# foubari/ratio_guided_Multimodal_FM

Measured on AMD Instinct MI355X. Metric: paired images/sec (MNIST32+SVHN, 100 Euler steps), higher is better.
Workload: dtype f32; 1 GPU; MNIST32 (1x32x32) + SVHN (3x32x32) pair, mc_feng guidance 0.5, 100 Euler steps, N_mc=256, batch 512 per GPU (BASELINE configs[2]; configs[3] at 8 GPUs); global_batch=512, parallelism=rows sharded over 1 rank(s); all_gather(MC set) + gather(outputs), step=one full sampling call (MC pre-phase + ratio + guided Euler loop + gather)

## Files before the change

### ratio_guided_multimodal_fm_amd/csrc/conv_mfma_hx2w.hip

```cpp
#include <stdlib.h>

#include <type_traits>

#include "conv_hx2_common.h"

namespace rgfm {

__global__ void hx2w_filter_transform_kernel(const float* w, float* u, int Cout, int Cin) {
  const size_t total = (size_t)Cout * Cin;
  for (size_t i = blockIdx.x * (size_t)blockDim.x + threadIdx.x; i < total; i += (size_t)gridDim.x * blockDim.x) {
    const float* g = w + i * 9;
    float t[4][3];
    for (int j = 0; j < 3; ++j) {
      t[0][j] = g[j];
      t[1][j] = 0.5f * (g[j] + g[3 + j] + g[6 + j]);
      t[2][j] = 0.5f * (g[j] - g[3 + j] + g[6 + j]);
      t[3][j] = g[6 + j];
    }
    for (int r = 0; r < 4; ++r) {
      u[i * 16 + r * 4 + 0] = t[r][0];
      u[i * 16 + r * 4 + 1] = 0.5f * (t[r][0] + t[r][1] + t[r][2]);
      u[i * 16 + r * 4 + 2] = 0.5f * (t[r][0] - t[r][1] + t[r][2]);
      u[i * 16 + r * 4 + 3] = t[r][2];
    }
  }
}

__device__ __forceinline__ void hx2w_split1(float v, unsigned short& h, unsigned short& l) {
  unsigned ph, pl;
  hsplit2(v, 0.f, ph, pl);
  h = (unsigned short)(ph & 0xffffu), l = (unsigned short)(pl & 0xffffu);
}

__global__ void hx2w_pack_kernel(const float* u, unsigned short* out, const float* hq, int Cout, int Cin) {
  const float sw = hq[2];
  const int nch = Cin / 16;
  const size_t total = (size_t)Cout * Cin * 16;
  for (size_t i = blockIdx.x * (size_t)blockDim.x + threadIdx.x; i < total; i += (size_t)gridDim.x * blockDim.x) {
    const int kk = (int)(i & 7), lane = (int)((i >> 3) & 63), nt = (int)((i >> 9) & 1), pos = (int)((i >> 10) & 15);
    const size_t r = i >> 14;
    const int ch = (int)(r % nch), cb = (int)(r / nch);
    const int co = cb * 64 + nt * 32 + (lane & 31), ci = ch * 16 + (lane >> 5) * 8 + kk;
    unsigned short h, l;
    hx2w_split1(sw * u[((size_t)co * Cin + ci) * 16 + pos], h, l);
    const size_t o = ((((((size_t)cb * nch + ch) * 16 + pos) * 2 + nt) * 2) * 64 + lane) * 8 + kk;
    out[o] = h, out[o + 512] = l;
  }
}

void hx2_scale_launch(const float* w, size_t n, float* hq, hipStream_t s);
void launch_pack_conv_hx2w(const float* w, void* out, float* hq, float* tmp, int Cout, int Cin, hipStream_t s) {
  hipLaunchKernelGGL(hx2w_filter_transform_kernel, dim3(256), dim3(256), 0, s, w, tmp, Cout, Cin);
  hx2_scale_launch(tmp, (size_t)Cout * Cin * 16, hq, s);
  hipLaunchKernelGGL(hx2w_pack_kernel, dim3(256), dim3(256), 0, s, tmp, (unsigned short*)out, hq, Cout, Cin);
}

constexpr int HX2W_RREC = 80;

template <int WL2>
__global__ __launch_bounds__(512, 2) void conv_mfma_hx2w_kernel(const ConvArgs a, const int num_tiles) {
  constexpr int W = 1 << WL2, TH = 256 / W, TX = W / 2, WR = W + 2, HR = TH + 2, HALO = HR * WR;
  constexpr int PW = WR / 2, PH = HR / 2, PSZ = PW * PH;
  constexpr int RBYTES = ((4 * PSZ * HX2W_RREC + 1023) / 1024) * 1024;
  constexpr int MAXIT = (HALO * 4 + 511) / 512;
  extern __shared__ __attribute__((aligned(16))) char smw[];
  char* const sV = smw + RBYTES;
  float* const sTab = reinterpret_cast<float*>(smw + 128 * 1024 + 64 * 32 * 8);

  const int tid = threadIdx.x, lane = tid & 63, wave = __builtin_amdgcn_readfirstlane((int)threadIdx.x >> 6);
  const int l31 = lane & 31, hp = lane >> 5;
  const TileGeom g = a.g;
  const int H = g.H;
  const int tile = (int)blockIdx.x;
  const int b0 = tile / g.tps, row0 = (tile - b0 * g.tps) * TH;
  const int cb = (int)blockIdx.y;
  const int cin = a.C0 + a.C1, nch = cin / KC;
  (void)num_tiles;

  const int q4 = tid & 3;
  int poff[MAXIT], rdst[MAXIT];
  unsigned okmask = 0u;
#pragma unroll
  for (int j = 0; j < MAXIT; ++j) {
    const int it = tid + 512 * j;
    poff[j] = 0, rdst[j] = 4 * PSZ * HX2W_RREC + q4 * 16;
    if (it < HALO * 4) {
      const int hpx = it >> 2;
      const int hy = hpx / WR, hx = hpx - hy * WR;
      const int y = row0 + hy - 1, x = hx - 1;
      const int rec = ((hy & 1) * 2 + (hx & 1)) * PSZ + (hy >> 1) * PW + (hx >> 1);
      rdst[j] = rec * HX2W_RREC + q4 * 16;
      if (y >= 0 && y < H && x >= 0 && x < W) {
        okmask |= 1u << j;
        poff[j] = (b0 * H + y) * W + x;
      }
    }
  }
  static_assert(RBYTES >= 4 * PSZ * HX2W_RREC + 64, "room for the trash record");
  f32x4 ra[MAXIT];
  float hmax = 0.f;
  auto issue_a = [&](int c) {
    const int ch0 = c * KC;
    const bool first = ch0 < a.C0;
    const float* src = first ? a.in0 + ch0 : a.in1 + (ch0 - a.C0);
    const unsigned cs = (unsigned)(first ? a.C0 : a.C1);
#pragma unroll
    for (int j = 0; j < MAXIT; ++j)
      ra[j] = *(const hx_gf32x4*)(src + (size_t)(__umul24((unsigned)poff[j], cs) + (unsigned)(q4 * 4)));
  };
  issue_a(0);

  if (a.gn_stats0) {
    const GnLane gn_lane(wave, lane, gn_waves_log2(cin >> 3), cin >> 3);
    if (gn_lane.row == 0) gn_table_row(a, gn_lane, b0, true, sTab, HX_SA);
  } else {
    for (int c = tid; c < cin; c += 512) {
      const float2 e = *reinterpret_cast<const float2*>(a.ab + ((size_t)b0 * cin + c) * 2);
      float2 o;
      o.x = HX_SA * e.x, o.y = HX_SA * e.y;
      *reinterpret_cast<float2*>(sTab + 2 * c) = o;
    }
  }

  auto commit_a = [&](int c) {
    const char* ep = reinterpret_cast<const char*>(sTab) + (c * KC + 4 * q4) * 8;
    const f32x4 e0 = *reinterpret_cast<const f32x4*>(ep), e1 = *reinterpret_cast<const f32x4*>(ep + 16);
    char* const rb = smw;
#pragma unroll
    for (int j = 0; j < MAXIT; ++j) {
      f32x4 v = ra[j];
      v.x = silu_scaled(fmaf(e0.x, v.x, e0.y));
      v.y = silu_scaled(fmaf(e0.z, v.y, e0.w));
      v.z = silu_scaled(fmaf(e1.x, v.z, e1.y));
      v.w = silu_scaled(fmaf(e1.z, v.w, e1.w));
      const float keep = ((okmask >> j) & 1u) ? 1.f : 0.f;
      v = v * keep;
      hmax = hx_absmax3(v.x, v.y, hmax);
      hmax = hx_absmax3(v.z, v.w, hmax);
      *reinterpret_cast<f32x4*>(rb + rdst[j]) = v;
    }
  };

  const int grp = wave >> 2;
  const int tt = tid & 63, tq = wave & 3;
  const int tty = tt / TX, ttx = tt - tty * TX;
  const int rbase = (tty * PW + ttx) * HX2W_RREC + tq * 16;
  const int vkey = (tt >> 2) & 3;
  const int vdst_h = grp * (8 * 64 * HRW) + tt * HRW + (((tq >> 1) ^ vkey) & 3) * 16 + (tq & 1) * 8;
  const int vdst_l = grp * (8 * 64 * HRW) + tt * HRW + (((2 + (tq >> 1)) ^ vkey) & 3) * 16 + (tq & 1) * 8;

  int aofs[2][2];
#pragma unroll
  for (int mt = 0; mt < 2; ++mt)
#pragma unroll
    for (int pl = 0; pl < 2; ++pl) aofs[mt][pl] = (32 * mt + l31) * HRW + (((2 * pl + hp) ^ ((l31 >> 2) & 3)) & 3) * 16;
  const char* const wbase = reinterpret_cast<const char*>(a.wpkw) + (size_t)cb * nch * (16 * 4096) + (size_t)(2 * wave) * 4096 + lane * 16;
  f16x8 bfr[2][2][2];
  auto issue_b = [&](int c) {
    const char* p = wbase + (size_t)c * (16 * 4096);
#pragma unroll
    for (int pi = 0; pi < 2; ++pi)
#pragma unroll
      for (int nt = 0; nt < 2; ++nt)
#pragma unroll
        for (int pl = 0; pl < 2; ++pl)
          bfr[pi][nt][pl] = __builtin_bit_cast(f16x8, *(const hx_gf32x4*)(p + pi * 4096 + nt * 2048 + pl * 1024));
  };

  f32x16 acc[2][2][2];
#pragma unroll
  for (int pi = 0; pi < 2; ++pi)
#pragma unroll
    for (int mt = 0; mt < 2; ++mt)
#pragma unroll
      for (int nt = 0; nt < 2; ++nt)
#pragma unroll
        for (int r = 0; r < 16; ++r) acc[pi][mt][nt][r] = 0.f;

  auto transform = [&](int c) {
    const char* const rb = smw + rbase;
    auto rd = [&](int i, int j) -> f32x4 {
      const int off = (((i & 1) * 2 + (j & 1)) * PSZ + (i >> 1) * PW + (j >> 1)) * HX2W_RREC;
      return *reinterpret_cast<const f32x4*>(rb + off);
    };
    struct P2 {
      hx_f32x2 lo, hi;
    };
    auto ld = [&](int i, int j) -> P2 {
      const f32x4 v = rd(i, j);
      return P2{hx_f32x2{v.x, v.y}, hx_f32x2{v.z, v.w}};
    };
    auto sub = [](const P2& x, const P2& y) { return P2{x.lo - y.lo, x.hi - y.hi}; };
    auto add = [](const P2& x, const P2& y) { return P2{x.lo + y.lo, x.hi + y.hi}; };
    P2 t0[4], t1[4];
    if (grp == 0) {
#pragma unroll
      for (int j = 0; j < 4; ++j) {
        const P2 d0 = ld(0, j), d1 = ld(1, j), d2 = ld(2, j);
        t0[j] = sub(d0, d2), t1[j] = add(d1, d2);
      }
    } else {
#pragma unroll
      for (int j = 0; j < 4; ++j) {
        const P2 d1 = ld(1, j), d2 = ld(2, j), d3 = ld(3, j);
        t0[j] = sub(d2, d1), t1[j] = sub(d1, d3);
      }
    }
#pragma unroll
    for (int r = 0; r < 2; ++r) {
      const P2* t = r ? t1 : t0;
      const P2 v[4] = {sub(t[0], t[2]), add(t[1], t[2]), sub(t[2], t[1]), sub(t[1], t[3])};
#pragma unroll
      for (int cc = 0; cc < 4; ++cc) {
        unsigned h0, l0, h1, l1;
        hsplit2(v[cc].lo.x, v[cc].lo.y, h0, l0);
        hsplit2(v[cc].hi.x, v[cc].hi.y, h1, l1);
        const hx_u32x2 ph = {h0, h1}, pl = {l0, l1};
        *reinterpret_cast<hx_u32x2*>(sV + vdst_h + (r * 4 + cc) * (64 * HRW)) = ph;
        *reinterpret_cast<hx_u32x2*>(sV + vdst_l + (r * 4 + cc) * (64 * HRW)) = pl;
      }
    }
  };
  auto multiply = [&]() {
#pragma unroll
    for (int pi = 0; pi < 2; ++pi) {
      const char* vp = sV + (2 * wave + pi) * (64 * HRW);
      f16x8 af[2][2];
#pragma unroll
      for (int mt = 0; mt < 2; ++mt)
#pragma unroll
        for (int pl = 0; pl < 2; ++pl) af[mt][pl] = *reinterpret_cast<const f16x8*>(vp + aofs[mt][pl]);
      hx_mma3<2>(acc[pi], af, bfr[pi]);
    }
  };

  __syncthreads();
#pragma unroll 1
  for (int c = 0; c < nch; ++c) {
    commit_a(c);
    issue_b(c);
    __syncthreads();
    issue_a(c + 1 < nch ? c + 1 : c);
    transform(c);
    __syncthreads();
    multiply();
  }
  if (!(4.f * hmax < HX_BIG)) atomicOr(a.range_flag, 1u);

  const float qinv = a.hqw[1];
  float* const sE = reinterpret_cast<float*>(smw);
  float* const sS = reinterpret_cast<float*>(smw + 128 * 1024);
  const bool sample_ok = b0 < a.B;
  const int et = tid >> 3, ecq = tid & 7;
  const int ety = et / TX, etx = et - ety * TX;
  const size_t pix = ((size_t)b0 * H + row0 + 2 * ety) * W + 2 * etx;
  auto pass = [&](auto nt_tag) {
    constexpr int nt = decltype(nt_tag)::value;
    __syncthreads();
#pragma unroll
    for (int pi = 0; pi < 2; ++pi)
#pragma unroll
      for (int mt = 0; mt < 2; ++mt) {
        float* e = sE + ((size_t)(2 * wave + pi) * 64 + 32 * mt) * 32 + l31;
#pragma unroll
        for (int r = 0; r < 16; ++r) e[((r & 3) + 8 * (r >> 2) + 4 * hp) * 32] = acc[pi][mt][nt][r];
      }
    __syncthreads();
    const int c = cb * 64 + nt * 32 + 4 * ecq;
    f32x4 add = *reinterpret_cast<const f32x4*>(a.bias + c);
    if (a.temb && sample_ok)
      add += *reinterpret_cast<const f32x4*>(a.temb + ((size_t)(a.temb_per_row ? b0 : 0) + (a.step_ptr ? (size_t)*a.step_ptr : 0)) * a.temb_stride + c);
    f32x4 mm[16];
#pragma unroll
    for (int p = 0; p < 16; ++p) mm[p] = *reinterpret_cast<const f32x4*>(sE + ((size_t)(p * 64 + et) * 32 + 4 * ecq));
    f32x4 s0[4], s1[4];
#pragma unroll
    for (int cc = 0; cc < 4; ++cc) {
      s0[cc] = mm[cc] + mm[4 + cc] + mm[8 + cc];
      s1[cc] = mm[4 + cc] - mm[8 + cc] - mm[12 + cc];
    }
    f32x4 y[4] = {s0[0] + s0[1] + s0[2], s0[1] - s0[2] - s0[3], s1[0] + s1[1] + s1[2], s1[1] - s1[2] - s1[3]};
#pragma unroll
    for (int i = 0; i < 4; ++i) {
      y[i] = y[i] * qinv + add;
      const size_t o = (pix + (i >> 1) * W + (i & 1)) * a.Cout + c;
      if (a.res_mode == 1 && sample_ok) y[i] += *reinterpret_cast<const f32x4*>(a.res0 + o);
      if (sample_ok) *reinterpret_cast<f32x4*>(a.out + o) = y[i];
    }
    if (a.small_check && a.range_flag && sample_ok) {
      float m = 0.f;
#pragma unroll
      for (int i = 0; i < 4; ++i) m = hx_absmax3(y[i].x, y[i].y, hx_absmax3(y[i].z, y[i].w, m));
      hx_small_flag(a.range_flag, m);
    }
    {
      const f32x4 mean = ((y[0] + y[1]) + (y[2] + y[3])) * 0.25f;
      f32x4 m2 = {0.f, 0.f, 0.f, 0.f};
#pragma unroll
      for (int i = 0; i < 4; ++i) m2 += (y[i] - mean) * (y[i] - mean);
      const f32x4 lo = {mean.x, m2.x, mean.y, m2.y}, hi = {mean.z, m2.z, mean.w, m2.w};
      float* sp = sS + ((size_t)et * 32 + 4 * ecq) * 2;
      *reinterpret_cast<f32x4*>(sp) = lo;
      *reinterpret_cast<f32x4*>(sp + 4) = hi;
    }
    __syncthreads();
    if (tid < 128 && a.stats_out && sample_ok) {
      const int part = tid >> 5, co = tid & 31;
      float2 sv[16];
#pragma unroll
      for (int k = 0; k < 16; ++k) sv[k] = *reinterpret_cast<const float2*>(sS + ((size_t)(16 * part + k) * 32 + co) * 2);
      double mean = 0.0, m2 = 0.0;
#pragma unroll
      for (int k = 0; k < 16; ++k) {
        const double d = (double)sv[k].x - mean;
        mean += d * (1.0 / (double)(k + 1));
        m2 += (double)sv[k].y + d * d * (4.0 * (double)k / (double)(k + 1));
      }
      const int gpart = (tile - b0 * g.tps) * 4 + part;
      float2 o;
      o.x = (float)mean, o.y = (float)m2;
      *reinterpret_cast<float2*>(a.stats_out + (((size_t)b0 * g.nparts + gpart) * a.Cout + cb * 64 + nt * 32 + co) * 2) = o;
    }
  };
  pass(std::integral_constant<int, 0>{});
  pass(std::integral_constant<int, 1>{});
}

static size_t hx2w_lds_bytes(const ConvArgs& a) {
  return (size_t)128 * 1024 + 64 * 32 * 8 + (size_t)(a.C0 + a.C1) * 8;
}

bool conv_hx2w_supported(const ConvArgs& a, int mode) {
  if (mode != CONV_S1 || !a.wpkw || !a.hqw || !a.range_flag) return false;
  const TileGeom& g = a.g;
  if (g.spt != 1 || (g.W != 16 && g.W != 32) || g.th * g.W != 256 || g.H % g.th != 0) return false;
  if (a.Hin != g.H || a.Win != g.W) return false;
  if (a.Cout % 64 != 0 || (a.C0 + a.C1) % KC != 0 || a.C0 % KC != 0) return false;
  if (a.res_mode == 2 || a.fin_ab || a.pout || a.pin0 || a.ep_scale || !a.out) return false;
  if (a.res_mode == 1 && a.R0 != a.Cout) return false;
  if (a.gn_stats0) {
    const int cin = a.C0 + a.C1;
    if (cin < 32 || cin % 8 != 0 || cin > 256 || a.gn_nparts0 > 16 || a.gn_g.nparts > 16) return false;
  } else if (!a.ab) {
    return false;
  }
  const size_t px = (size_t)a.B * a.g.HW;
  if (px >= (1u << 24) || px * (size_t)(a.C0 > a.Cout ? a.C0 : a.Cout) >= (1ull << 32)) return false;
  return hx2w_lds_bytes(a) <= 160 * 1024;
}

#define HX2W_FOR_ALL(X) X(4) X(5)

int conv_hx2w_init() {
  int rc = 0;
#define RAISEWN(WL) rc |= raise_lds_limit(&conv_mfma_hx2w_kernel<WL>, 160 * 1024);
  HX2W_FOR_ALL(RAISEWN)
#undef RAISEWN
  return rc;
}

bool launch_conv_hx2w(const ConvArgs& a, int mode, hipStream_t s) {
  if (mode != CONV_S1) return false;
  const int tiles = geom_num_tiles(a.g, a.B);
  const dim3 grid(tiles, a.Cout / 64);
  const size_t lds = hx2w_lds_bytes(a);
  const int wl = a.g.W == 16 ? 4 : 5;
#define LAUNCHWN(WL) \
  if (wl == (WL)) { hipLaunchKernelGGL((conv_mfma_hx2w_kernel<WL>), grid, dim3(512), lds, s, a, tiles); return true; }
  HX2W_FOR_ALL(LAUNCHWN)
#undef LAUNCHWN
  return false;
}
#undef HX2W_FOR_ALL

}
```

### ratio_guided_multimodal_fm_amd/csrc/rgfm_host.h

```cpp
#pragma once
#include "../../include/rgfm.h"

#include <hip/hip_runtime.h>

#include <algorithm>
#include <cmath>
#include <cstdarg>
#include <cstdio>
#include <cstdlib>
#include <cstring>
#include <string>
#include <vector>

#include "rgfm_kernels.h"

using namespace rgfm;

inline thread_local std::string g_err;

inline int fail(int code, const char* fmt, ...) {
  char buf[512];
  va_list ap;
  va_start(ap, fmt);
  vsnprintf(buf, sizeof(buf), fmt, ap);
// ... 89 lines not shown

struct Bump {
  char* base = nullptr;
  size_t off = 0;
  size_t cap = 0;
  bool dry = true;
  bool overflow = false;
  Bump() = default;
  Bump(void* ws, size_t ws_bytes) : base((char*)ws), cap(ws_bytes), dry(false) {}
  unsigned* u(size_t n) { return reinterpret_cast<unsigned*>(f(n)); }
  float* f(size_t nfloats) {
    const size_t bytes = (nfloats * sizeof(float) + 255) & ~(size_t)255;
    const size_t o = off;
    off += bytes;
    if (dry) return nullptr;
    if (off > cap) {
      overflow = true;
      return reinterpret_cast<float*>(base);
    }
    return reinterpret_cast<float*>(base + o);
  }
};

struct Tensor {
  float* data = nullptr;
  float* stats = nullptr;
  int C = 0, S = 0;
  void* p = nullptr;
  bool p_valid = false;
};

struct Cursor {
  size_t off = 0;
  size_t take(size_t n) {
    const size_t r = off;
    off += n;
    return r;
  }
};

struct HxImage {
  size_t off = 0;
  int hq = 0;
  bool present = false;
  bool ok = false;
  bool usable() const { return present && ok; }
};

struct ConvW {
  size_t w_raw = 0, b = 0;
  size_t w_pk = 0;
  size_t w_bx3 = 0;
  int cin = 0, cout = 0, taps = 9;
  HxImage hx;
  HxImage hx9;
  HxImage wino;
  HxImage t2;
};

struct WeightLayout {
  size_t n_params = 0, n_packed = 0, n_packed3 = 0, n_packedh = 0;
  int n_hq = 0;
};

struct Planner {
  Cursor raw, pk, p3, ph;
  int nhq = 0;
  HxImage image(size_t n_fp16, const HxImage* same_scale = nullptr) {
    HxImage i;
    i.off = ph.take(n_fp16), i.hq = same_scale ? same_scale->hq : nhq++, i.present = true;
    return i;
  }
  ConvW conv(int cin, int cout, int taps) {
    ConvW w;
    w.cin = cin, w.cout = cout, w.taps = taps;
    w.w_raw = raw.take((size_t)cout * cin * taps);
    w.b = raw.take(cout);
    w.w_pk = pk.take((size_t)cout * cin * taps);
    w.w_bx3 = p3.take((size_t)cout * cin * taps * 3);
    w.hx = image((size_t)cout * cin * taps * 2);
    return w;
  }
  WeightLayout layout() const { return {raw.off, pk.off, p3.off, ph.off, nhq}; }
};

struct ResW {
  int cin = 0, cout = 0;
  size_t n1w, n1b, n2w, n2b, tw, tb;
  ConvW c1, c2, sk;
  bool has_skip = false;
  int temb_off = 0;
};

inline int nt32_of(int cout) { return (cout % 64 == 0) ? 2 : 1; }

inline bool on_gfx950() {
  int dev = 0;
  if (hipGetDevice(&dev) != hipSuccess) return false;
  hipDeviceProp_t p;
  if (hipGetDeviceProperties(&p, dev) != hipSuccess) return false;
  return strncmp(p.gcnArchName, "gfx950", 6) == 0;
}

enum { CONV_ARITH_HX2 = 0, CONV_ARITH_BX3 = 1, CONV_ARITH_F32 = 2 };
struct Modes {
  int conv = CONV_ARITH_HX2;
  bool overlap = true, fuse_fin = true, gn_consumer = true;
  bool pipelined = true;
  bool quad = true;
  bool c8 = true;
  bool s2 = true;
  bool pfmt = true;
  bool wino = false;
  bool up_t2 = true;
  bool rev_hx2 = true;
  bool prephase = true;
  bool graph = false;
};
inline thread_local Modes g_modes;
inline void refresh_modes() {
  Modes m;
  const char* e = getenv("RGFM_CONV");
  if (e && strcmp(e, "bx3") == 0) m.conv = CONV_ARITH_BX3;
  else if (e && strcmp(e, "f32") == 0) m.conv = CONV_ARITH_F32;
  e = getenv("RGFM_OVERLAP");
  m.overlap = !(e && e[0] == '0');
  e = getenv("RGFM_FUSE_FIN");
  m.fuse_fin = !(e && e[0] == '0');
  e = getenv("RGFM_GN");
  m.gn_consumer = !(e && strcmp(e, "table") == 0);
  e = getenv("RGFM_HX2P");
  m.pipelined = !(e && e[0] == '0');
  e = getenv("RGFM_HX2Q");
  m.quad = !(e && e[0] == '0');
  e = getenv("RGFM_HX2S");
  m.s2 = !(e && e[0] == '0');
  e = getenv("RGFM_HX2C");
  m.c8 = !(e && e[0] == '0');
  e = getenv("RGFM_HX2D");
  m.pfmt = !(e && e[0] == '0');
  g_conv_tuning.hx2d_cut = e && e[0] == '1' ? 1 : (e && e[0] == '2' ? 2 : 3);
  e = getenv("RGFM_WINO");
  m.wino = e && e[0] == '1';
  e = getenv("RGFM_UP_T2");
  m.up_t2 = !(e && e[0] == '0');
  e = getenv("RGFM_REV_HX2");
  m.rev_hx2 = !(e && e[0] == '0');
  e = getenv("RGFM_GRAPH");
  m.graph = e && e[0] == '1';
  e = getenv("RGFM_PREPHASE_PRIO");
  m.prephase = !(e && e[0] == '0');
  g_modes = m;
  e = getenv("RGFM_WINO_W32");
  g_conv_tuning.wino_w32 = e ? atoi(e) : 0;
  g_conv_tuning.s2_f32 = getenv("RGFM_S2_F32") != nullptr;
  g_conv_tuning.f32_simple = getenv("RGFM_CONV_SIMPLE") != nullptr;
}

struct ModeScope {
  int saved;
  explicit ModeScope(int handle_mode) : saved(g_modes.conv) {
    if (handle_mode >= 0) g_modes.conv = handle_mode;
  }
  ~ModeScope() { g_modes.conv = saved; }
};

constexpr int MAX_DEVICES = 16;
struct DevState {
  bool init = false;
  int num_cus = 256;
  hipStream_t side = nullptr;
  void* zeros = nullptr;
  hipEvent_t fork = nullptr, join = nullptr;
  hipEvent_t pre_pace = nullptr;
  hipStream_t main = nullptr;
  hipEvent_t main_fork = nullptr, main_join = nullptr;
  hipEvent_t graph_done = nullptr;
  std::vector<std::pair<hipGraphExec_t, hipGraph_t>> graphs;
};
inline DevState g_dev[MAX_DEVICES];

inline DevState* cur_dev() {
  int dev = 0;
  if (hipGetDevice(&dev) != hipSuccess || dev < 0 || dev >= MAX_DEVICES) return nullptr;
  return g_dev[dev].init ? &g_dev[dev] : nullptr;
}

inline int ensure_init() {
  if (!on_gfx950()) return fail(RGFM_ENODEVICE, "librgfm_hip needs a gfx950 (MI355X) device; none is current");
  int dev = 0;
  HIP_TRY(hipGetDevice(&dev));
  if (dev < 0 || dev >= MAX_DEVICES) return fail(RGFM_EINVAL, "device ordinal %d out of range (max %d)", dev, MAX_DEVICES - 1);
  DevState& d = g_dev[dev];
  if (!d.init) {
    int rc = guid_apply_init();
    for (const ConvKernel& k : CONV_KERNELS) rc |= k.init();
    if (rc != 0) return fail(RGFM_EHIP, "hipFuncSetAttribute(MaxDynamicSharedMemorySize) failed");
    hipDeviceProp_t p;
    if (hipGetDeviceProperties(&p, dev) == hipSuccess) d.num_cus = p.multiProcessorCount;
    const char* e = getenv("RGFM_HX2P_HALF");
    g_conv_tuning.hx2p_half = e ? atoi(e) : d.num_cus;
    HIP_TRY(hipStreamCreateWithFlags(&d.side, hipStreamNonBlocking));
    HIP_TRY(hipMalloc(&d.zeros, 256));
    HIP_TRY(hipMemset(d.zeros, 0, 256));
    HIP_TRY(hipEventCreateWithFlags(&d.fork, hipEventDisableTiming));
    HIP_TRY(hipEventCreateWithFlags(&d.join, hipEventDisableTiming));
    HIP_TRY(hipEventCreateWithFlags(&d.graph_done, hipEventDisableTiming));
    HIP_TRY(hipStreamCreateWithFlags(&d.main, hipStreamNonBlocking));
    HIP_TRY(hipEventCreateWithFlags(&d.main_fork, hipEventDisableTiming));
    HIP_TRY(hipEventCreateWithFlags(&d.main_join, hipEventDisableTiming));
    HIP_TRY(hipEventCreateWithFlags(&d.pre_pace, hipEventDisableTiming));
    d.init = true;
  }
  return RGFM_OK;
}

inline bool hx2w_pays(const ConvArgs& c) {
  return c.wpkw != nullptr && c.C0 + c.C1 >= 128 && (!g_conv_tuning.wino_w32 || c.g.W == 32);
}

inline int conv_route(const ConvArgs& c, int mode) {
  if (c.pin0) return RGFM_ROUTE_HX2D;
  const bool hx2 = g_modes.conv == CONV_ARITH_HX2, pipe = hx2 && g_modes.pipelined;
  if (pipe && g_modes.wino && hx2w_pays(c) && conv_hx2w_supported(c, mode)) return RGFM_ROUTE_HX2W;
  if (pipe && g_modes.s2 && conv_hx2s_supported(c, mode)) return RGFM_ROUTE_HX2S;
  if (pipe && g_modes.c8 && conv_hx2c_supported(c, mode)) return RGFM_ROUTE_HX2C;
  if (pipe && g_modes.quad && conv_hx2q_supported(c, mode)) return RGFM_ROUTE_HX2Q;
  if (pipe && conv_hx2p_supported(c, mode)) return RGFM_ROUTE_HX2P;
  if (hx2 && conv_hx2_supported(c, mode)) return RGFM_ROUTE_HX2;
  if (g_modes.conv != CONV_ARITH_F32 && conv_bx3_supported(c, mode)) return RGFM_ROUTE_BX3;
  return RGFM_ROUTE_F32;
}

inline bool p_producer_ok(const ConvArgs& c, int mode) {
  if (!g_modes.pfmt) return false;
  const int route = conv_route(c, mode);
  if (route == RGFM_ROUTE_HX2C) return true;
  return route == RGFM_ROUTE_HX2P && mode == CONV_S1 && c.g.W == 16 && c.g.H == 16 && c.g.spt == 1 && c.g.tps == 1 &&
         (c.Cout == 64 || c.Cout == 128 || c.Cout == 256) && !c.ep_scale && !c.fin_ab;
}

inline bool launch_conv_on(int route, const ConvArgs& c, int mode, hipStream_t s) {
  const ConvKernel& k = CONV_KERNELS[route];
  if (k.launch(c, mode, s)) return true;
  fail(RGFM_EINVAL, "no %s instantiation for mode %d, Cout %d, %d x %d raster, res_mode %d", k.name, mode, c.Cout, c.g.H, c.g.W, c.res_mode);
  return false;
}

inline void launch_conv(const ConvArgs& c, int mode, hipStream_t s, int* routes = nullptr) {
  const int route = conv_route(c, mode);
  if (routes) {
    routes[route] += 1;
    if (mode == CONV_T2) routes[RGFM_ROUTE_T2] += 1;
  }
  launch_conv_on(route, c, mode, s);
}



inline int read_flag_word(unsigned* word, int* flagged, int reset, hipStream_t s) {
  if (!flagged) return fail(RGFM_EINVAL, "null output");
  *flagged = 0;
  if (!word) return RGFM_OK;
  unsigned v = 0;
  HIP_TRY(hipMemcpyAsync(&v, word, sizeof(v), hipMemcpyDeviceToHost, s));
  HIP_TRY(hipStreamSynchronize(s));
  *flagged = (int)v;
  if (reset && v) HIP_TRY(hipMemsetAsync(word, 0, sizeof(v), s));
  return RGFM_OK;
}
inline int alloc_flag_word(unsigned** word) {
  HIP_TRY(hipMalloc(word, 256));
  HIP_TRY(hipMemset(*word, 0, 256));
  return RGFM_OK;
}
inline int check_conv_mode(int mode) {
  if (mode < -1 || mode > CONV_ARITH_F32) return fail(RGFM_EINVAL, "conv mode must be RGFM_CONV_DEFAULT, _HX2, _BX3 or _F32");
  return RGFM_OK;
}


struct WeightStore : WeightLayout {
  float* params = nullptr;
  float* packed = nullptr;
  unsigned short* packed3 = nullptr;
  unsigned short* packedh = nullptr;
  float* hq = nullptr;
  unsigned* range_flag = nullptr;
  int conv_mode = -1;

  int alloc(const float* params_dev, bool with_range_flag, hipStream_t s) {
    if (hipMalloc(&params, n_params * sizeof(float)) != hipSuccess) return fail(RGFM_ENOMEM, "hipMalloc(params)");
    if (hipMalloc(&packed, (n_packed + 4) * sizeof(float)) != hipSuccess) return fail(RGFM_ENOMEM, "hipMalloc(packed)");
    if (hipMalloc(&packedh, (n_packedh + 8) * sizeof(unsigned short)) != hipSuccess) return fail(RGFM_ENOMEM, "hipMalloc(packedh)");
    if (hipMalloc(&hq, ((size_t)n_hq * 4 + 4) * sizeof(float)) != hipSuccess) return fail(RGFM_ENOMEM, "hipMalloc(hq)");
    if (with_range_flag && alloc_flag_word(&range_flag) != RGFM_OK) return fail(RGFM_ENOMEM, "hipMalloc(range flag)");
    if (n_packed3 && hipMalloc(&packed3, (n_packed3 + 8) * sizeof(unsigned short)) != hipSuccess)
      return fail(RGFM_ENOMEM, "hipMalloc(packed3)");
    if (hipMemcpyAsync(params, params_dev, n_params * sizeof(float), hipMemcpyDeviceToDevice, s) != hipSuccess)
      return fail(RGFM_EHIP, "hipMemcpyAsync(params)");
    return RGFM_OK;
  }
  void free() {
    for (void* p : {(void*)params, (void*)packed, (void*)packed3, (void*)packedh, (void*)hq, (void*)range_flag})
      if (p) (void)hipFree(p);
  }
};

inline int read_hx_flags(const WeightStore& st, const std::vector<HxImage*>& images, hipStream_t s) {
  std::vector<float> host((size_t)st.n_hq * 4);
  if (hipMemcpyAsync(host.data(), st.hq, host.size() * sizeof(float), hipMemcpyDeviceToHost, s) != hipSuccess ||
      hipStreamSynchronize(s) != hipSuccess)
    return fail(RGFM_EHIP, "reading the fp16 scale records failed");
  for (HxImage* i : images) i->ok = host[(size_t)i->hq * 4 + 3] != 0.f;
  return RGFM_OK;
}

inline bool norm_params_ok(const std::vector<float>& host, size_t gw, size_t gb, int C) {
  float mg = 0.f, mb = 0.f;
  for (int i = 0; i < C; ++i) mg = std::max(mg, std::fabs(host[gw + i])), mb = std::max(mb, std::fabs(host[gb + i]));
  if (!(mg <= 3.0e38f) || !(mb <= 3.0e38f)) return false;
  const float hi = 8.f * mg + mb, lo = std::max(mg, mb);
  return hi < 1024.f && lo >= 0.015625f;
}

struct NormGate {
  size_t gamma, beta;
  int C;
  HxImage* image;
};

inline int demote_by_norms(const WeightStore& st, const std::vector<NormGate>& gates, hipStream_t s) {
  std::vector<float> host(st.n_params);
  if (hipMemcpyAsync(host.data(), st.params, host.size() * sizeof(float), hipMemcpyDeviceToHost, s) != hipSuccess ||
      hipStreamSynchronize(s) != hipSuccess)
    return fail(RGFM_EHIP, "reading the parameters back failed");
  for (const NormGate& g : gates)
    if (!norm_params_ok(host, g.gamma, g.beta, g.C)) g.image->ok = false;
  return RGFM_OK;
}


struct rgfm_unet : WeightStore {
  rgfm_unet_desc d;
  float* freqs = nullptr;
  TimeLinear* lin_dev = nullptr;
  float* wtmp = nullptr;
  int mc = 0, temb = 0, nlin = 0, temb_total = 0;
  size_t te0w, te0b, te2w, te2b, icw, icb, onw, onb, ocw, ocb;
  size_t ocw_pk = 0;
  std::vector<ResW> enc, mid, dec;
  std::vector<ConvW> down, up;
  int final_ch = 0;
  bool trace = false;
  int wino_convs = 0;
  int p_handovers = 0;
  int routes[RGFM_ROUTE_SLOTS] = {};
  struct Act {
    float* data;
    int C, S;
    bool nchw;
  };
  std::vector<Act> acts;
};


inline size_t plan_unet(const rgfm_unet_desc& d, rgfm_unet* h) {
  Planner P;
  Cursor& c = P.raw;
  const int mc = d.model_channels, temb = 4 * mc;
  std::vector<ResW> enc, mid, dec;
// ... 530 lines not shown
```

### ratio_guided_multimodal_fm_amd/csrc/rgfm_kernels.h

```cpp
#pragma once
#include <hip/hip_runtime.h>
#include <stddef.h>
#include <stdint.h>

#include "../../include/rgfm.h"

namespace rgfm {

constexpr int KC = 16;
constexpr int LDP = 20;

struct TileGeom {
  int H, W, HW;
  int spt;
  int th;
  int tps;
  int nparts;
};

__host__ __device__ inline TileGeom make_geom(int H, int W) {
  TileGeom g;
  g.H = H;
  g.W = W;
  g.HW = H * W;
// ... 16 lines not shown
__host__ __device__ inline int geom_num_tiles(const TileGeom& g, int B) {
  return g.spt == 1 ? B * g.tps : (B + g.spt - 1) / g.spt;
}

__host__ __device__ inline int geom_part_count(const TileGeom& g, int part) {
  if (g.spt != 1) return g.HW;
  const int tile = part >> 2, w = part & 3;
  int rows = g.H - tile * g.th;
  if (rows > g.th) rows = g.th;
  int n = rows * g.W - 64 * w;
  return n < 0 ? 0 : (n > 64 ? 64 : n);
}

enum ConvMode { CONV_S1 = 0, CONV_S2 = 1, CONV_UP2 = 2, CONV_T2 = 3 };

struct ConvArgs {
  const float* in0;
  const float* in1;
  int C0, C1;
  int Hin, Win;
  const float* ab;
  const float* gn_stats0;
  const float* gn_stats1;
  const float* gn_gamma;
  const float* gn_beta;
  int gn_nparts0;
  TileGeom gn_g;
  const unsigned* in_amax;
  const void* pin0;
  const void* zeros;
  void* pout;
  const float* pn_gamma;
  const float* pn_beta;
  const float* wpk;
  const void* wpk3;
  const void* wskip3;
  const void* wpkh;
  const void* wskiph;
  const void* wpkh9;
  const float* hq;
  const float* hq_skip;
  unsigned* range_flag;
  int small_check;
  const float* bias;
  const float* temb;
  int temb_stride;
  int temb_per_row;
  const int* step_ptr;
  int res_mode;
  const float* res0;
  const float* res1;
  int R0, R1;
  const float* wskip;
  const float* skip_bias;
  const float* ep_scale;
  const float* ep_shift;
  int ep_nosilu;
  float* out;
  float* stats_out;
  float* fin_ab;
  unsigned* fin_counter;
  int fin_expected;
  const float* fin_stats1;
  int fin_C1;
  const float* fin_gamma;
  const float* fin_beta;
  const void* wpkw;
  const float* hqw;
  int B, Cout;
  TileGeom g;
  int halo_px;
};

inline int conv_halo_px(const ConvArgs& a) { return a.g.spt * (a.g.th + 2) * (a.g.W + 2); }
inline int conv_block_channels(int Cout) { return Cout % 128 == 0 ? 128 : (Cout % 64 == 0 ? 64 : 32); }
template <class Kernel>
inline int raise_lds_limit(Kernel* kernel, int bytes) {
  return (int)hipFuncSetAttribute(reinterpret_cast<const void*>(kernel), hipFuncAttributeMaxDynamicSharedMemorySize, bytes);
}

struct ConvInArgs {
  const float* x;
  const float* w;
  const float* bias;
  const float* ep_scale;
  const float* ep_shift;
  int ep_nosilu;
  float* out;
  float* stats_out;
  int B, C0;
  TileGeom g;
  unsigned* range_flag;
  int small_check;
};

struct ConvOutArgs {
  const float* in;
  const float* ab;
  const float* w;
  const float* bias;
  float* v_out;
  float* x_state;
  const float* x_base;
  float dt;
  int B, Cin;
  TileGeom g;
  int halo_px;
};

struct GnFinalizeArgs {
  const float* stats0;
  const float* stats1;
  int C0, C1, groups;
  const float* gamma;
  const float* beta;
  float* ab;
  int B;
  TileGeom g;
  int rep;
  float* mr;
};

struct TimeLinear {
  int w_off, b_off, cout, out_off;
};

struct TimeEmbedArgs {
  const float* params;
  const float* freqs;
  int mc, temb;
  int te0w, te0b, te2w, te2b;
  const TimeLinear* lin;
  int nlin;
  int total;
  const float* t_dev;
  int num_steps, step_begin;
  float* table;
  float* emb_out;
};


struct ConvTuning {
  int hx2p_half = 256;
  int hx2p_w4 = 0;
  int hx2q_min = 1024;
  int hx2q_target = 512;
  int hx2q_tpw = 0;
  int hx2q_cut = 0;
  int hx2q_all = 0;
  int hx2s_on = 1;
  int hx2c_on = 1;
  int hx2c_all = 0;
  int hx2d_cut = 3;
  int wino_w32 = 0;
  bool s2_f32 = false;
  bool f32_simple = false;
};
inline ConvTuning g_conv_tuning;

int conv_fin_expected(const ConvArgs& a, int mode);

int conv_mfma_init();
bool launch_conv_mfma(const ConvArgs& a, int mode, hipStream_t s);
size_t conv_mfma_lds_bytes(const ConvArgs& a);

bool conv_bx3_supported(const ConvArgs& a, int mode);
bool conv_bx3_gn_supported(const ConvArgs& a, int mode);
int conv_bx3_init();
bool launch_conv_bx3(const ConvArgs& a, int mode, hipStream_t s);
void launch_pack_conv_bx3(const float* w, void* out, int Cout, int Cin, int taps, hipStream_t s);
void launch_pack_deconv_bx3(const float* w, void* out, int Cin, int Cout, hipStream_t s);
void launch_pack_conv_bx3_s2(const float* w, void* out, int Cout, int Cin, hipStream_t s);

bool conv_hx2_supported(const ConvArgs& a, int mode);
bool conv_hx2_gn_supported(const ConvArgs& a, int mode);
int conv_hx2_init();
bool launch_conv_hx2(const ConvArgs& a, int mode, hipStream_t s);
void launch_pack_conv_hx2(const float* w, void* out, float* hq, int Cout, int Cin, int taps, int mode, hipStream_t s);
void launch_up2_as_deconv(const float* w, float* k, int Cout, int Cin, hipStream_t s);

bool conv_hx2p_supported(const ConvArgs& a, int mode);
int conv_hx2p_init();
bool launch_conv_hx2p(const ConvArgs& a, int mode, hipStream_t s);

bool conv_hx2q_supported(const ConvArgs& a, int mode);
int conv_hx2q_init();
bool launch_conv_hx2q(const ConvArgs& a, int mode, hipStream_t s);

bool conv_hx2s_supported(const ConvArgs& a, int mode);
int conv_hx2s_init();
bool launch_conv_hx2s(const ConvArgs& a, int mode, hipStream_t s);

bool conv_hx2c_supported(const ConvArgs& a, int mode);
int conv_hx2c_init();
bool launch_conv_hx2c(const ConvArgs& a, int mode, hipStream_t s);

bool conv_hx2d_supported(const ConvArgs& a, int mode);
int conv_hx2d_init();
bool launch_conv_hx2d(const ConvArgs& a, int mode, hipStream_t s);
void launch_hx_presplit(const float* in, const float* ab, void* pout, int B, int HW, int C, hipStream_t s);

bool conv_hx2w_supported(const ConvArgs& a, int mode);
int conv_hx2w_init();
bool launch_conv_hx2w(const ConvArgs& a, int mode, hipStream_t s);
void hx2_scale_launch(const float* w, size_t n, float* hq, hipStream_t s);
void launch_pack_conv_hx2w(const float* w, void* out, float* hq, float* tmp, int Cout, int Cin, hipStream_t s);

struct ConvKernel {
  const char* name;
  int (*init)();
  bool (*launch)(const ConvArgs& a, int mode, hipStream_t s);
};
inline constexpr ConvKernel CONV_KERNELS[RGFM_ROUTE_COUNT] = {
    {"hx2d", conv_hx2d_init, launch_conv_hx2d},
    {"hx2w", conv_hx2w_init, launch_conv_hx2w},
    {"hx2s", conv_hx2s_init, launch_conv_hx2s},
    {"hx2c", conv_hx2c_init, launch_conv_hx2c},
    {"hx2q", conv_hx2q_init, launch_conv_hx2q},
    {"hx2p", conv_hx2p_init, launch_conv_hx2p},
    {"hx2", conv_hx2_init, launch_conv_hx2},
    {"bx3", conv_bx3_init, launch_conv_bx3},
    {"f32", conv_mfma_init, launch_conv_mfma},
};
static_assert(RGFM_ROUTE_HX2D == 0 && RGFM_ROUTE_HX2W == 1 && RGFM_ROUTE_HX2S == 2 && RGFM_ROUTE_HX2C == 3 && RGFM_ROUTE_HX2Q == 4 &&
                  RGFM_ROUTE_HX2P == 5 && RGFM_ROUTE_HX2 == 6 && RGFM_ROUTE_BX3 == 7 && RGFM_ROUTE_F32 == 8,
              "CONV_KERNELS is written in RGFM_ROUTE_* order");

void launch_conv_in(const ConvInArgs& a, int cin, hipStream_t s);
void launch_conv_out(const ConvOutArgs& a, int cimg, hipStream_t s);
void launch_pack_conv_out(const float* w, float* out, int cimg, int Cin, hipStream_t s);
void launch_gn_finalize(const GnFinalizeArgs& a, hipStream_t s);
void launch_time_embed(const TimeEmbedArgs& a, int nt, hipStream_t s);
void launch_pack_conv(const float* w, float* out, int Cout, int Cin, int taps, int nt32, hipStream_t s);
void launch_pack_deconv(const float* w, float* out, int Cin, int Cout, int nt32, hipStream_t s);
void launch_permute_cols(const float* w, float* out, int rows, int C, int P, hipStream_t s);
void launch_permute_rows(const float* w, const float* b, float* wout, float* bout, int C, int P, int K, hipStream_t s);
void launch_fm_time_embed(const float* t_dev, int t_count, int num_steps, int step, const float* freqs, float* out,
                          int B, int dim, int stride, int col0, hipStream_t s);
void launch_nhwc_to_nchw(const float* in, float* out, int B, int C, int HW, hipStream_t s);
void launch_range_low_check(const float* in, int B, int HW, int C, unsigned* flag, hipStream_t s);

void launch_pool2(const float* in, const float* ab, float* out, int B, int H, int W, int C, hipStream_t s);
void launch_avgpool(const float* in, const float* ab, float* out, int B, int HW, int C, hipStream_t s);
void launch_linear_mfma(const float* x, const float* w, const float* b, float* y, int rows, int in,
                        int out, int x_stride, int y_stride, hipStream_t s);
void launch_linear_mfma_splitk(const float* x, const float* ab, int C, const float* w, const float* b, float* y,
                               float* part, int splits, int rows, int in, int out, int y_stride, hipStream_t s);
void launch_layernorm_silu(float* x, const float* w, const float* b, int rows, int n, hipStream_t s);
void launch_cross_ln_silu(const float* ux, const float* uy, const float* bias, const float* w, const float* b, float* out,
                          long long row0, int rows, int ny, int n, hipStream_t s);
void launch_cond_ln_silu(const float* ctx, const float* ut, const float* w, const float* b, float* u, float* a, int rows, int n,
                         hipStream_t s);
void launch_ratio_head(const float* x, const float* w, const float* b, float* out, int rows, int n,
                       int loss, int what, hipStream_t s);
void launch_bn_fold(const float* w, const float* b, const float* rm, const float* rv, float* scale,
                    float* shift, int C, hipStream_t s);

void launch_conv_weight_transpose(const float* w, float* wt, int Co, int Ci, hipStream_t s);
void launch_transpose2d(const float* w, float* wt, int rows, int cols, hipStream_t s);
void launch_fill(float* p, float v, size_t n, hipStream_t s);
void launch_fill_ab_identity(float* ab, size_t n_pairs, hipStream_t s);
void launch_grad_act(const float* g, const float* z, const float* scale, float* gz, int B, int S, int C, int mode, hipStream_t s,
                     unsigned* amax = nullptr);
void launch_grad_act_gn(const float* g, const float* z, const float* ab, float* gu, int B, int S, int C, int mode, hipStream_t s);
void launch_gn_bwd(float* gu, const float* z, const float* gamma, const float* mr, int B, int HW, int C, int groups, hipStream_t s);
void launch_conv_bwd_img(const float* gz, const float* w, float* gimg, int B, int S, int Co, int cimg, hipStream_t s);
void launch_layernorm_silu_bwd(const float* u, const float* gy, const float* w, const float* b, float* gu, int rows, int n, hipStream_t s);
void launch_ratio_head_bwd(const float* score, const float* w, float* gh, float* log_ratio, int rows, int n, int loss, hipStream_t s);
void launch_euler_grad(float* x, const float* v, const float* g, size_t n, float gamma, float dt, hipStream_t s,
                       const float* base = nullptr);

struct GuidanceArgs {
  const float* x;
  const float* y;
  float* vx;
  float* vy;
  const float* mc_x1;
  const float* mc_y1;
  const float* mc_ratios;
  int ratio_stride;
  int B, N, dx, dy;
  float tf, s2, cden, g1, g2;
  double* dist;
  int slice_len, nsx, nsy;
  const float* sched;
  const int* step_ptr;
  float* weights_out;
  float* wbuf;
  float* wsum;
  float* diag_rec;
  float* x_state;
  float* y_state;
  const float* x_base;
  const float* y_base;
  float dt;
};
constexpr int RGFM_GUID_SLICES = 8;
void launch_guid_logp(const GuidanceArgs& a, hipStream_t s);
void launch_guid_weights(const GuidanceArgs& a, hipStream_t s);
void launch_guid_apply(const GuidanceArgs& a, hipStream_t s);
int guid_apply_init();
void launch_euler(float* x, const float* v, size_t n, float dt, hipStream_t s);
void launch_step_inc(int* step, hipStream_t s);
void launch_guid_schedule(float* sched, int step_begin, int ns, int num_steps, hipStream_t s);
void launch_diag_wstats(const float* w, int B, int N, float* rec, hipStream_t s);
void launch_diag_rownorm(const float* v, int B, int D, float* rec, int slot, hipStream_t s);

// ... 104 lines not shown
```

Measured before the change: 543.2 paired images/sec.

## Add 128-channel-wide Winograd conv tile variant with halved spatial tile

Templates the Winograd hx2 conv body on a CUT flag. When Cout is a multiple of 128, each workgroup covers 128 output channels over 32 spatial tiles instead of 64 channels over 64 tiles, so each B-fragment load is reused over more channels and the grid is reshaped to match. The input transform is split so each wave group computes one row, and the 3-term MFMA product is written out explicitly. New env knobs control the channel-cut width, the minimum Cin and the width filter for routing. The trade-offs are a different amount of halo overhead per tile and more register pressure from four N accumulators.

```diff
diff --git a/ratio_guided_multimodal_fm_amd/csrc/conv_mfma_hx2w.hip b/ratio_guided_multimodal_fm_amd/csrc/conv_mfma_hx2w.hip
--- a/ratio_guided_multimodal_fm_amd/csrc/conv_mfma_hx2w.hip
+++ b/ratio_guided_multimodal_fm_amd/csrc/conv_mfma_hx2w.hip
@@ -57,25 +57,30 @@
 
 constexpr int HX2W_RREC = 80;
 
-template <int WL2>
-__global__ __launch_bounds__(512, 2) void conv_mfma_hx2w_kernel(const ConvArgs a, const int num_tiles) {
-  constexpr int W = 1 << WL2, TH = 256 / W, TX = W / 2, WR = W + 2, HR = TH + 2, HALO = HR * WR;
+template <int WL2, int CUT>
+__device__ __forceinline__ void hx2w_body(const ConvArgs& a) {
+  constexpr int NTL = CUT ? 32 : 64;
+  constexpr int MT = NTL / 32, NT = CUT ? 4 : 2;
+  constexpr int CB = 32 * NT, EC = CB / 2, NTP = NT / 2;
+  constexpr int WPT = 64 / NTL;
+  constexpr int W = 1 << WL2, TH = 4 * NTL / W, TX = W / 2, WR = W + 2, HR = TH + 2, HALO = HR * WR;
   constexpr int PW = WR / 2, PH = HR / 2, PSZ = PW * PH;
   constexpr int RBYTES = ((4 * PSZ * HX2W_RREC + 1023) / 1024) * 1024;
   constexpr int MAXIT = (HALO * 4 + 511) / 512;
+  static_assert(MT * NT == 4 && NTL * EC == 2048 && TH % 2 == 0, "2 x 4 accumulators per wave; E is 128 KB per pass");
+  static_assert(RBYTES + 16 * NTL * HRW <= 128 * 1024, "R and V fit inside E");
   extern __shared__ __attribute__((aligned(16))) char smw[];
   char* const sV = smw + RBYTES;
-  float* const sTab = reinterpret_cast<float*>(smw + 128 * 1024 + 64 * 32 * 8);
+  float* const sTab = reinterpret_cast<float*>(smw + 128 * 1024 + NTL * EC * 8);
 
   const int tid = threadIdx.x, lane = tid & 63, wave = __builtin_amdgcn_readfirstlane((int)threadIdx.x >> 6);
   const int l31 = lane & 31, hp = lane >> 5;
   const TileGeom g = a.g;
   const int H = g.H;
-  const int tile = (int)blockIdx.x;
-  const int b0 = tile / g.tps, row0 = (tile - b0 * g.tps) * TH;
+  const int wg = (int)blockIdx.x, tile = wg / WPT;
+  const int b0 = tile / g.tps, wgs = wg - b0 * g.tps * WPT, row0 = wgs * TH;
   const int cb = (int)blockIdx.y;
   const int cin = a.C0 + a.C1, nch = cin / KC;
-  (void)num_tiles;
 
   const int q4 = tid & 3;
   int poff[MAXIT], rdst[MAXIT];
@@ -141,44 +146,52 @@
     }
   };
 
-  const int grp = wave >> 2;
-  const int tt = tid & 63, tq = wave & 3;
+  const int grp = CUT ? wave >> 1 : wave >> 2;
+  const int tt = tid & (NTL - 1), tq = CUT ? (wave & 1) * 2 + hp : wave & 3;
   const int tty = tt / TX, ttx = tt - tty * TX;
   const int rbase = (tty * PW + ttx) * HX2W_RREC + tq * 16;
   const int vkey = (tt >> 2) & 3;
-  const int vdst_h = grp * (8 * 64 * HRW) + tt * HRW + (((tq >> 1) ^ vkey) & 3) * 16 + (tq & 1) * 8;
-  const int vdst_l = grp * (8 * 64 * HRW) + tt * HRW + (((2 + (tq >> 1)) ^ vkey) & 3) * 16 + (tq & 1) * 8;
-
-  int aofs[2][2];
-#pragma unroll
-  for (int mt = 0; mt < 2; ++mt)
+  constexpr int VGRP = (CUT ? 4 : 8) * NTL * HRW;
+  const int vdst_h = grp * VGRP + tt * HRW + (((tq >> 1) ^ vkey) & 3) * 16 + (tq & 1) * 8;
+  const int vdst_l = grp * VGRP + tt * HRW + (((2 + (tq >> 1)) ^ vkey) & 3) * 16 + (tq & 1) * 8;
+
+  int aofs[MT][2];
+#pragma unroll
+  for (int mt = 0; mt < MT; ++mt)
 #pragma unroll
     for (int pl = 0; pl < 2; ++pl) aofs[mt][pl] = (32 * mt + l31) * HRW + (((2 * pl + hp) ^ ((l31 >> 2) & 3)) & 3) * 16;
-  const char* const wbase = reinterpret_cast<const char*>(a.wpkw) + (size_t)cb * nch * (16 * 4096) + (size_t)(2 * wave) * 4096 + lane * 16;
-  f16x8 bfr[2][2][2];
+  const size_t wblk = (size_t)nch * (16 * 4096);
+  const char* const wbase = reinterpret_cast<const char*>(a.wpkw) + (size_t)(cb * (NT / 2)) * wblk + (size_t)(2 * wave) * 4096 + lane * 16;
+  f16x8 bfr[2][NT][2];
   auto issue_b = [&](int c) {
     const char* p = wbase + (size_t)c * (16 * 4096);
 #pragma unroll
     for (int pi = 0; pi < 2; ++pi)
 #pragma unroll
-      for (int nt = 0; nt < 2; ++nt)
+      for (int nt = 0; nt < NT; ++nt)
 #pragma unroll
         for (int pl = 0; pl < 2; ++pl)
-          bfr[pi][nt][pl] = __builtin_bit_cast(f16x8, *(const hx_gf32x4*)(p + pi * 4096 + nt * 2048 + pl * 1024));
-  };
-
-  f32x16 acc[2][2][2];
+          bfr[pi][nt][pl] = __builtin_bit_cast(f16x8, *(const hx_gf32x4*)(p + (nt >> 1) * wblk + pi * 4096 + (nt & 1) * 2048 + pl * 1024));
+  };
+
+  f32x16 acc[2][MT][NT];
 #pragma unroll
   for (int pi = 0; pi < 2; ++pi)
 #pragma unroll
-    for (int mt = 0; mt < 2; ++mt)
-#pragma unroll
-      for (int nt = 0; nt < 2; ++nt)
+    for (int mt = 0; mt < MT; ++mt)
+#pragma unroll
+      for (int nt = 0; nt < NT; ++nt)
 #pragma unroll
         for (int r = 0; r < 16; ++r) acc[pi][mt][nt][r] = 0.f;
 
   auto transform = [&](int c) {
     const char* const rb = smw + rbase;
+    int vdl = vdst_l;
+    if constexpr (CUT) {
+      vdl = vdst_h;
+      asm volatile("" : "+v"(vdl));
+      vdl ^= 32;
+    }
     auto rd = [&](int i, int j) -> f32x4 {
       const int off = (((i & 1) * 2 + (j & 1)) * PSZ + (i >> 1) * PW + (j >> 1)) * HX2W_RREC;
       return *reinterpret_cast<const f32x4*>(rb + off);
@@ -193,7 +206,21 @@
     auto sub = [](const P2& x, const P2& y) { return P2{x.lo - y.lo, x.hi - y.hi}; };
     auto add = [](const P2& x, const P2& y) { return P2{x.lo + y.lo, x.hi + y.hi}; };
     P2 t0[4], t1[4];
-    if (grp == 0) {
+    if constexpr (CUT) {
+      if (grp == 0) {
+#pragma unroll
+        for (int j = 0; j < 4; ++j) t0[j] = sub(ld(0, j), ld(2, j));
+      } else if (grp == 1) {
+#pragma unroll
+        for (int j = 0; j < 4; ++j) t0[j] = add(ld(1, j), ld(2, j));
+      } else if (grp == 2) {
+#pragma unroll
+        for (int j = 0; j < 4; ++j) t0[j] = sub(ld(2, j), ld(1, j));
+      } else {
+#pragma unroll
+        for (int j = 0; j < 4; ++j) t0[j] = sub(ld(1, j), ld(3, j));
+      }
+    } else if (grp == 0) {
 #pragma unroll
       for (int j = 0; j < 4; ++j) {
         const P2 d0 = ld(0, j), d1 = ld(1, j), d2 = ld(2, j);
@@ -207,7 +234,7 @@
       }
     }
 #pragma unroll
-    for (int r = 0; r < 2; ++r) {
+    for (int r = 0; r < (CUT ? 1 : 2); ++r) {
       const P2* t = r ? t1 : t0;
       const P2 v[4] = {sub(t[0], t[2]), add(t[1], t[2]), sub(t[2], t[1]), sub(t[1], t[3])};
 #pragma unroll
@@ -216,21 +243,36 @@
         hsplit2(v[cc].lo.x, v[cc].lo.y, h0, l0);
         hsplit2(v[cc].hi.x, v[cc].hi.y, h1, l1);
         const hx_u32x2 ph = {h0, h1}, pl = {l0, l1};
-        *reinterpret_cast<hx_u32x2*>(sV + vdst_h + (r * 4 + cc) * (64 * HRW)) = ph;
-        *reinterpret_cast<hx_u32x2*>(sV + vdst_l + (r * 4 + cc) * (64 * HRW)) = pl;
+        *reinterpret_cast<hx_u32x2*>(sV + vdst_h + (r * 4 + cc) * (NTL * HRW)) = ph;
+        *reinterpret_cast<hx_u32x2*>(sV + vdl + (r * 4 + cc) * (NTL * HRW)) = pl;
       }
     }
   };
   auto multiply = [&]() {
+    int aol = aofs[0][1];
+    if constexpr (CUT) {
+      aol = aofs[0][0];
+      asm volatile("" : "+v"(aol));
+      aol ^= 32;
+    }
 #pragma unroll
     for (int pi = 0; pi < 2; ++pi) {
-      const char* vp = sV + (2 * wave + pi) * (64 * HRW);
-      f16x8 af[2][2];
-#pragma unroll
-      for (int mt = 0; mt < 2; ++mt)
-#pragma unroll
-        for (int pl = 0; pl < 2; ++pl) af[mt][pl] = *reinterpret_cast<const f16x8*>(vp + aofs[mt][pl]);
-      hx_mma3<2>(acc[pi], af, bfr[pi]);
+      const char* vp = sV + (2 * wave + pi) * (NTL * HRW);
+      f16x8 af[MT][2];
+#pragma unroll
+      for (int mt = 0; mt < MT; ++mt)
+#pragma unroll
+        for (int pl = 0; pl < 2; ++pl) af[mt][pl] = *reinterpret_cast<const f16x8*>(vp + (CUT && pl ? aol : aofs[mt][pl]));
+      if constexpr (CUT) {
+        constexpr int PA[3] = {1, 0, 0}, PB[3] = {0, 1, 0};
+#pragma unroll
+        for (int q = 0; q < 3; ++q)
+#pragma unroll
+          for (int nt = 0; nt < NT; ++nt)
+            acc[pi][0][nt] = __builtin_amdgcn_mfma_f32_32x32x16_f16(af[0][PA[q]], bfr[pi][nt][PB[q]], acc[pi][0][nt], 0, 0, 0);
+      } else {
+        hx_mma3<2>(acc[pi], af, bfr[pi]);
+      }
     }
   };
 
@@ -251,28 +293,34 @@
   float* const sE = reinterpret_cast<float*>(smw);
   float* const sS = reinterpret_cast<float*>(smw + 128 * 1024);
   const bool sample_ok = b0 < a.B;
-  const int et = tid >> 3, ecq = tid & 7;
+  constexpr int QPT = EC / 4;
+  int tide = (int)threadIdx.x;
+  asm volatile("" : "+v"(tide));
+  const int l31e = tide & 31, hpe = (tide >> 5) & 1;
+  const int et = tide / QPT, ecq = tide % QPT;
   const int ety = et / TX, etx = et - ety * TX;
   const size_t pix = ((size_t)b0 * H + row0 + 2 * ety) * W + 2 * etx;
-  auto pass = [&](auto nt_tag) {
-    constexpr int nt = decltype(nt_tag)::value;
+  auto pass = [&](auto ps_tag) {
+    constexpr int ps = decltype(ps_tag)::value;
     __syncthreads();
 #pragma unroll
     for (int pi = 0; pi < 2; ++pi)
 #pragma unroll
-      for (int mt = 0; mt < 2; ++mt) {
-        float* e = sE + ((size_t)(2 * wave + pi) * 64 + 32 * mt) * 32 + l31;
-#pragma unroll
-        for (int r = 0; r < 16; ++r) e[((r & 3) + 8 * (r >> 2) + 4 * hp) * 32] = acc[pi][mt][nt][r];
-      }
+      for (int mt = 0; mt < MT; ++mt)
+#pragma unroll
+        for (int ntp = 0; ntp < NTP; ++ntp) {
+          float* e = sE + ((size_t)(2 * wave + pi) * NTL + 32 * mt) * EC + 32 * ntp + l31e;
+#pragma unroll
+          for (int r = 0; r < 16; ++r) e[((r & 3) + 8 * (r >> 2) + 4 * hpe) * EC] = acc[pi][mt][ps * NTP + ntp][r];
+        }
     __syncthreads();
-    const int c = cb * 64 + nt * 32 + 4 * ecq;
+    const int c = cb * CB + ps * EC + 4 * ecq;
     f32x4 add = *reinterpret_cast<const f32x4*>(a.bias + c);
     if (a.temb && sample_ok)
       add += *reinterpret_cast<const f32x4*>(a.temb + ((size_t)(a.temb_per_row ? b0 : 0) + (a.step_ptr ? (size_t)*a.step_ptr : 0)) * a.temb_stride + c);
     f32x4 mm[16];
 #pragma unroll
-    for (int p = 0; p < 16; ++p) mm[p] = *reinterpret_cast<const f32x4*>(sE + ((size_t)(p * 64 + et) * 32 + 4 * ecq));
+    for (int p = 0; p < 16; ++p) mm[p] = *reinterpret_cast<const f32x4*>(sE + ((size_t)(p * NTL + et) * EC + 4 * ecq));
     f32x4 s0[4], s1[4];
 #pragma unroll
     for (int cc = 0; cc < 4; ++cc) {
@@ -299,16 +347,16 @@
 #pragma unroll
       for (int i = 0; i < 4; ++i) m2 += (y[i] - mean) * (y[i] - mean);
       const f32x4 lo = {mean.x, m2.x, mean.y, m2.y}, hi = {mean.z, m2.z, mean.w, m2.w};
-      float* sp = sS + ((size_t)et * 32 + 4 * ecq) * 2;
+      float* sp = sS + ((size_t)et * EC + 4 * ecq) * 2;
       *reinterpret_cast<f32x4*>(sp) = lo;
       *reinterpret_cast<f32x4*>(sp + 4) = hi;
     }
     __syncthreads();
-    if (tid < 128 && a.stats_out && sample_ok) {
-      const int part = tid >> 5, co = tid & 31;
+    if (tid < (NTL / 16) * EC && a.stats_out && sample_ok) {
+      const int part = tid / EC, co = tid % EC;
       float2 sv[16];
 #pragma unroll
-      for (int k = 0; k < 16; ++k) sv[k] = *reinterpret_cast<const float2*>(sS + ((size_t)(16 * part + k) * 32 + co) * 2);
+      for (int k = 0; k < 16; ++k) sv[k] = *reinterpret_cast<const float2*>(sS + ((size_t)(16 * part + k) * EC + co) * 2);
       double mean = 0.0, m2 = 0.0;
 #pragma unroll
       for (int k = 0; k < 16; ++k) {
@@ -316,14 +364,30 @@
         mean += d * (1.0 / (double)(k + 1));
         m2 += (double)sv[k].y + d * d * (4.0 * (double)k / (double)(k + 1));
       }
-      const int gpart = (tile - b0 * g.tps) * 4 + part;
+      const int gpart = wgs * (NTL / 16) + part;
       float2 o;
       o.x = (float)mean, o.y = (float)m2;
-      *reinterpret_cast<float2*>(a.stats_out + (((size_t)b0 * g.nparts + gpart) * a.Cout + cb * 64 + nt * 32 + co) * 2) = o;
+      *reinterpret_cast<float2*>(a.stats_out + (((size_t)b0 * g.nparts + gpart) * a.Cout + cb * CB + ps * EC + co) * 2) = o;
     }
   };
   pass(std::integral_constant<int, 0>{});
   pass(std::integral_constant<int, 1>{});
+}
+
+template <int WL2>
+__global__ __launch_bounds__(512, 2) void conv_mfma_hx2w_kernel(const ConvArgs a, const int num_tiles) {
+  (void)num_tiles;
+  hx2w_body<WL2, 0>(a);
+}
+template <int WL2>
+__global__ __launch_bounds__(512, 2) void conv_mfma_hx2w128_kernel(const ConvArgs a, const int num_tiles) {
+  (void)num_tiles;
+  hx2w_body<WL2, 1>(a);
+}
+template <int WL2, int CUT>
+constexpr auto hx2w_kernel() {
+  if constexpr (CUT) return &conv_mfma_hx2w128_kernel<WL2>;
+  else return &conv_mfma_hx2w_kernel<WL2>;
 }
 
 static size_t hx2w_lds_bytes(const ConvArgs& a) {
@@ -349,11 +413,13 @@
   return hx2w_lds_bytes(a) <= 160 * 1024;
 }
 
-#define HX2W_FOR_ALL(X) X(4) X(5)
+static int hx2w_cut(const ConvArgs& a) { return a.Cout % 128 == 0 && g_conv_tuning.wino_cut != 64 ? 1 : 0; }
+
+#define HX2W_FOR_ALL(X) X(4, 0) X(5, 0) X(4, 1) X(5, 1)
 
 int conv_hx2w_init() {
   int rc = 0;
-#define RAISEWN(WL) rc |= raise_lds_limit(&conv_mfma_hx2w_kernel<WL>, 160 * 1024);
+#define RAISEWN(WL, CUT) rc |= raise_lds_limit(hx2w_kernel<WL, CUT>(), 160 * 1024);
   HX2W_FOR_ALL(RAISEWN)
 #undef RAISEWN
   return rc;
@@ -362,11 +428,12 @@
 bool launch_conv_hx2w(const ConvArgs& a, int mode, hipStream_t s) {
   if (mode != CONV_S1) return false;
   const int tiles = geom_num_tiles(a.g, a.B);
-  const dim3 grid(tiles, a.Cout / 64);
+  const int cut = hx2w_cut(a);
+  const dim3 grid(cut ? 2 * tiles : tiles, cut ? a.Cout / 128 : a.Cout / 64);
   const size_t lds = hx2w_lds_bytes(a);
   const int wl = a.g.W == 16 ? 4 : 5;
-#define LAUNCHWN(WL) \
-  if (wl == (WL)) { hipLaunchKernelGGL((conv_mfma_hx2w_kernel<WL>), grid, dim3(512), lds, s, a, tiles); return true; }
+#define LAUNCHWN(WL, CUT) \
+  if (wl == (WL) && cut == (CUT)) { hipLaunchKernelGGL((hx2w_kernel<WL, CUT>()), grid, dim3(512), lds, s, a, tiles); return true; }
   HX2W_FOR_ALL(LAUNCHWN)
 #undef LAUNCHWN
   return false;
diff --git a/ratio_guided_multimodal_fm_amd/csrc/rgfm_host.h b/ratio_guided_multimodal_fm_amd/csrc/rgfm_host.h
--- a/ratio_guided_multimodal_fm_amd/csrc/rgfm_host.h
+++ b/ratio_guided_multimodal_fm_amd/csrc/rgfm_host.h
@@ -265,7 +265,13 @@
   m.prephase = !(e && e[0] == '0');
   g_modes = m;
   e = getenv("RGFM_WINO_W32");
-  g_conv_tuning.wino_w32 = e ? atoi(e) : 0;
+  g_conv_tuning.wino_w = e && atoi(e) ? 32 : 0;
+  e = getenv("RGFM_WINO_W");
+  if (e) g_conv_tuning.wino_w = atoi(e);
+  e = getenv("RGFM_WINO_CUT");
+  g_conv_tuning.wino_cut = e && atoi(e) == 64 ? 64 : 128;
+  e = getenv("RGFM_WINO_CIN");
+  g_conv_tuning.wino_min_cin = e ? atoi(e) : 128;
   g_conv_tuning.s2_f32 = getenv("RGFM_S2_F32") != nullptr;
   g_conv_tuning.f32_simple = getenv("RGFM_CONV_SIMPLE") != nullptr;
 }
@@ -329,7 +335,7 @@
 }
 
 inline bool hx2w_pays(const ConvArgs& c) {
-  return c.wpkw != nullptr && c.C0 + c.C1 >= 128 && (!g_conv_tuning.wino_w32 || c.g.W == 32);
+  return c.wpkw != nullptr && c.C0 + c.C1 >= g_conv_tuning.wino_min_cin && (!g_conv_tuning.wino_w || c.g.W == g_conv_tuning.wino_w);
 }
 
 inline int conv_route(const ConvArgs& c, int mode) {
diff --git a/ratio_guided_multimodal_fm_amd/csrc/rgfm_kernels.h b/ratio_guided_multimodal_fm_amd/csrc/rgfm_kernels.h
--- a/ratio_guided_multimodal_fm_amd/csrc/rgfm_kernels.h
+++ b/ratio_guided_multimodal_fm_amd/csrc/rgfm_kernels.h
@@ -192,7 +192,9 @@
   int hx2c_on = 1;
   int hx2c_all = 0;
   int hx2d_cut = 3;
-  int wino_w32 = 0;
+  int wino_w = 0;
+  int wino_min_cin = 128;
+  int wino_cut = 128;
   bool s2_f32 = false;
   bool f32_simple = false;
 };
```

After: 542.6 paired images/sec (median of 2 runs). Within noise of the previous version (-0.1%).
